# howardlau1999/pytorch-ddp-template

Hardware: NVIDIA H100
Metric: samples/sec (whole box, device-timed, max over ranks) for ResNet-50 DDP at 1/2/4/8 H100 (higher is better)
Workload: dtype bf16; 1 GPU; model=resnet50, global_batch=32, per_gpu_batch=32, image_size=224, parallelism=dp1, loss=mse(dense one-hot target), optimizer=sgd lr1e-3 + clip_grad_norm 1000 + linear warmup/decay, transport=single, cuda_graph=True

## Files before the change

### b200ddp/csrc/batchnorm.cu

```cuda
#include "ops.h"
#include "drv.h"
#include "tc_primitives.cuh"

#include <algorithm>
#include <cstdlib>
#include <map>
#include <mutex>
#include <utility>

namespace b200 {
namespace {

constexpr int kBnThreads = 256;
constexpr int kVec = 8;

template <typename T> __device__ __forceinline__ void bn_load8(const T* p, float* f);
template <> __device__ __forceinline__ void bn_load8<__nv_bfloat16>(const __nv_bfloat16* p, float* f) {
  unpack8(*reinterpret_cast<const Bf16x8*>(p), f);
}
template <> __device__ __forceinline__ void bn_load8<float>(const float* p, float* f) {
  const float4 a = reinterpret_cast<const float4*>(p)[0], b = reinterpret_cast<const float4*>(p)[1];
  f[0] = a.x; f[1] = a.y; f[2] = a.z; f[3] = a.w; f[4] = b.x; f[5] = b.y; f[6] = b.z; f[7] = b.w;
}
template <typename T> __device__ __forceinline__ void bn_store8(T* p, const float* f);
// ... 233 lines not shown
  bn_wait_producer();
  if (cv * kVec >= C) return;
  bn_apply_rows<T>(x, residual, y, mask, scale, shift, C, cv, r0, r1, tyi, ty, relu);
}

template <typename T>
__device__ __forceinline__ void bn_bwd_apply_rows(const T* __restrict__ dy, const T* __restrict__ x, const unsigned char* __restrict__ y,
                                                  T* __restrict__ dx, T* __restrict__ dres, const float* __restrict__ save_mean,
                                                  const float* __restrict__ save_rstd, const float* __restrict__ gamma,
                                                  const float* __restrict__ coef, int C, int cv, int r0, int r1, int tyi, int ty, int relu);
template <typename T>
__device__ __forceinline__ void bn_bwd_apply_rows_coef(const T* __restrict__ dy, const T* __restrict__ x, const unsigned char* __restrict__ y,
                                                       T* __restrict__ dx, T* __restrict__ dres, const float* __restrict__ save_mean,
                                                       const float* __restrict__ save_rstd, const float* __restrict__ gamma,
                                                       const float* c1p, const float* c2p, int C, int cv, int r0, int r1, int tyi, int ty, int relu);

template <typename T, bool FUSED, bool PDL = false>
__global__ void __launch_bounds__(kBnThreads, 2) bn_bwd_reduce_kernel(const T* __restrict__ dy, const T* __restrict__ x, const unsigned char* __restrict__ y,
                                                                     int R, int C, int cvb, int ty, int relu, const float* __restrict__ save_mean,
                                                                     const float* __restrict__ save_rstd, float* __restrict__ partial,
                                                                     unsigned int* __restrict__ counters, float* __restrict__ dgamma,
                                                                     float* __restrict__ dbeta, float* __restrict__ coef ,
                                                                     const float* __restrict__ gamma, T* __restrict__ dx, T* __restrict__ dres) {
  extern __shared__ float smem[];
  __shared__ bool is_last;
  unsigned int* gen = counters + gridDim.x;
  unsigned int gen0 = 0;
  if (FUSED && threadIdx.x == 0) gen0 = *reinterpret_cast<volatile unsigned int*>(&gen[blockIdx.x]);
  const int tx = threadIdx.x % cvb, tyi = threadIdx.x / cvb;
  const int cv = blockIdx.x * cvb + tx;
  const int S = gridDim.y;
  const int rows_per = (R + S - 1) / S;
  const int r0 = blockIdx.y * rows_per, r1 = min(R, r0 + rows_per);
  float acc[2][kVec];
#pragma unroll
  for (int i = 0; i < kVec; ++i) { acc[0][i] = 0.f; acc[1][i] = 0.f; }
  if (cv * kVec < C) {
    float mean[kVec], rstd[kVec];
    bn_load8<float>(save_mean + cv * kVec, mean);
    bn_load8<float>(save_rstd + cv * kVec, rstd);
    const size_t col = (size_t)cv * kVec;
    int r = r0 + tyi;
    for (; r + ty < r1; r += 2 * ty) {
      float g[2][kVec], xv[2][kVec];
      unsigned int mk[2] = {0xffu, 0xffu};
#pragma unroll
      for (int u = 0; u < 2; ++u) {
        const size_t off = (size_t)(r + u * ty) * C + col;
        bn_load8<T>(dy + off, g[u]);
        bn_load8<T>(x + off, xv[u]);
        if (relu) mk[u] = y[(size_t)(r + u * ty) * (C / kVec) + cv];
      }
#pragma unroll
      for (int u = 0; u < 2; ++u)
#pragma unroll
        for (int i = 0; i < kVec; ++i) {
          const float gm = ((mk[u] >> i) & 1u) ? g[u][i] : 0.f;
          acc[0][i] += gm;
          acc[1][i] = fmaf(gm, (xv[u][i] - mean[i]) * rstd[i], acc[1][i]);
        }
    }
    for (; r < r1; r += ty) {
      float g[kVec], xv[kVec];
      const size_t off = (size_t)r * C + col;
      bn_load8<T>(dy + off, g);
      bn_load8<T>(x + off, xv);
      const unsigned int mk = relu ? y[(size_t)r * (C / kVec) + cv] : 0xffu;
#pragma unroll
      for (int i = 0; i < kVec; ++i) {
        const float gm = ((mk >> i) & 1u) ? g[i] : 0.f;
        acc[0][i] += gm;
        acc[1][i] = fmaf(gm, (xv[i] - mean[i]) * rstd[i], acc[1][i]);
      }
    }
  }
  if constexpr (PDL) bn_launch_dependents();
  reduce_rows<2>(acc, smem, tx, tyi, cvb, ty);
  const int width = cvb * kVec;
  const int c0 = blockIdx.x * width;
  for (int c = threadIdx.x; c < width; c += blockDim.x) {
    if (c0 + c < C) {
      partial[(size_t)(0 * S + blockIdx.y) * C + c0 + c] = smem[c];
      partial[(size_t)(1 * S + blockIdx.y) * C + c0 + c] = smem[ty * width + c];
    }
  }
  __threadfence();
  __syncthreads();
  if (threadIdx.x == 0) {
    const unsigned int ticket = atomicAdd(&counters[blockIdx.x], 1u);
    is_last = (ticket == (unsigned int)S - 1);
  }
  __syncthreads();
  if (!FUSED && !is_last) return;
  if (is_last) {
    __threadfence();
    const float inv_r = 1.f / (float)R;
    const int lanes = max(1, (int)blockDim.x / width);
    {
      const int c = threadIdx.x % width, l = threadIdx.x / width;
      float ps = 0.f, pq = 0.f;
      if (l < lanes && c0 + c < C) {
  #pragma unroll 4
        for (int k = l; k < S; k += lanes) { ps += __ldcg(&partial[(size_t)(0 * S + k) * C + c0 + c]); pq += __ldcg(&partial[(size_t)(1 * S + k) * C + c0 + c]); }
      }
      __syncthreads();
      if (l < lanes) { smem[l * width + c] = ps; smem[(lanes + l) * width + c] = pq; }
      __syncthreads();
    }
    for (int c = threadIdx.x; c < width; c += blockDim.x) {
      const int ch = c0 + c;
      if (ch >= C) continue;
      float s = 0.f, q = 0.f;
      for (int l = 0; l < lanes; ++l) { s += smem[l * width + c]; q += smem[(lanes + l) * width + c]; }
      dbeta[ch] = s;
      dgamma[ch] = q;
      coef[ch] = s * inv_r;
      coef[C + ch] = q * inv_r;
    }

    __syncthreads();
    if (threadIdx.x == 0) {
      counters[blockIdx.x] = 0u;
      if (FUSED) { __threadfence(); bn_st_release(&gen[blockIdx.x], gen0 + 1u); }
    }
  }
  if (!FUSED) return;
  if (!is_last && threadIdx.x == 0) bn_wait_generation(&gen[blockIdx.x], gen0);
  __syncthreads();
  if (cv * kVec < C) bn_bwd_apply_rows<T>(dy, x, y, dx, dres, save_mean, save_rstd, gamma, coef, C, cv, r0, r1, tyi, ty, relu);
}

template <typename T>
__device__ __forceinline__ void bn_bwd_apply_rows_coef(const T* __restrict__ dy, const T* __restrict__ x, const unsigned char* __restrict__ y,
                                                       T* __restrict__ dx, T* __restrict__ dres, const float* __restrict__ save_mean,
                                                       const float* __restrict__ save_rstd, const float* __restrict__ gamma,
                                                       const float* c1p, const float* c2p, int C, int cv, int r0, int r1, int tyi, int ty, int relu) {
  float ka[kVec], kb[kVec], kc[kVec];
  {
    float mean[kVec], rstd[kVec], gam[kVec], c1[kVec], c2[kVec];
    bn_load8<float>(save_mean + cv * kVec, mean);
    bn_load8<float>(save_rstd + cv * kVec, rstd);
    bn_load8<float>(gamma + cv * kVec, gam);
    bn_load8<float>(c1p, c1);
    bn_load8<float>(c2p, c2);
#pragma unroll
    for (int i = 0; i < kVec; ++i) {
      ka[i] = gam[i] * rstd[i];
      kb[i] = -ka[i] * rstd[i] * c2[i];
      kc[i] = -ka[i] * (c1[i] - mean[i] * rstd[i] * c2[i]);
    }
  }
  const size_t col = (size_t)cv * kVec;
  int r = r0 + tyi;
  for (; r + ty < r1; r += 2 * ty) {
    float g[2][kVec], xv[2][kVec];
    unsigned int mk[2] = {0xffu, 0xffu};
#pragma unroll
    for (int u = 0; u < 2; ++u) {
      const size_t off = (size_t)(r + u * ty) * C + col;
      bn_load8<T>(dy + off, g[u]);
      bn_load8<T>(x + off, xv[u]);
      if (relu) mk[u] = y[(size_t)(r + u * ty) * (C / kVec) + cv];
    }
#pragma unroll
    for (int u = 0; u < 2; ++u) {
      const size_t off = (size_t)(r + u * ty) * C + col;
      float o[kVec];
#pragma unroll
      for (int i = 0; i < kVec; ++i) {
        if (!((mk[u] >> i) & 1u)) g[u][i] = 0.f;
        o[i] = fmaf(ka[i], g[u][i], fmaf(kb[i], xv[u][i], kc[i]));
      }
      if (dres != nullptr) bn_store8<T>(dres + off, g[u]);
      bn_store8<T>(dx + off, o);
    }
  }
  for (; r < r1; r += ty) {
    const size_t off = (size_t)r * C + col;
    float g[kVec], xv[kVec], o[kVec];
    bn_load8<T>(dy + off, g);
    bn_load8<T>(x + off, xv);
    const unsigned int mk = relu ? y[(size_t)r * (C / kVec) + cv] : 0xffu;
#pragma unroll
    for (int i = 0; i < kVec; ++i) {
      if (!((mk >> i) & 1u)) g[i] = 0.f;
      o[i] = fmaf(ka[i], g[i], fmaf(kb[i], xv[i], kc[i]));
    }
    if (dres != nullptr) bn_store8<T>(dres + off, g);
    bn_store8<T>(dx + off, o);
  }
}

template <typename T>
__device__ __forceinline__ void bn_bwd_apply_rows(const T* __restrict__ dy, const T* __restrict__ x, const unsigned char* __restrict__ y,
                                                  T* __restrict__ dx, T* __restrict__ dres, const float* __restrict__ save_mean,
                                                  const float* __restrict__ save_rstd, const float* __restrict__ gamma,
                                                  const float* __restrict__ coef, int C, int cv, int r0, int r1, int tyi, int ty, int relu) {
  bn_bwd_apply_rows_coef<T>(dy, x, y, dx, dres, save_mean, save_rstd, gamma, coef + cv * kVec, coef + C + cv * kVec, C, cv, r0, r1, tyi, ty, relu);
}

template <typename T>
__global__ void __launch_bounds__(kBnThreads) bn_bwd_apply_kernel(const T* __restrict__ dy, const T* __restrict__ x, const unsigned char* __restrict__ y,
                                                                 T* __restrict__ dx, T* __restrict__ dres, const float* __restrict__ save_mean,
                                                                 const float* __restrict__ save_rstd, const float* __restrict__ gamma,
                                                                 const float* __restrict__ coef, int R, int C, int cvb, int ty, int relu) {
  const int tx = threadIdx.x % cvb, tyi = threadIdx.x / cvb;
  const int cv = blockIdx.x * cvb + tx;
  if (cv * kVec >= C) return;
  const int S = gridDim.y;
  const int rows_per = (R + S - 1) / S;
  const int r0 = blockIdx.y * rows_per, r1 = min(R, r0 + rows_per);
  bn_bwd_apply_rows<T>(dy, x, y, dx, dres, save_mean, save_rstd, gamma, coef, C, cv, r0, r1, tyi, ty, relu);
}

template <typename T>
__global__ void __launch_bounds__(kBnThreads) bn_bwd_apply_pdl_kernel(const T* __restrict__ dy, const T* __restrict__ x, const unsigned char* __restrict__ y,
                                                                     T* __restrict__ dx, T* __restrict__ dres, const float* __restrict__ save_mean,
                                                                     const float* __restrict__ save_rstd, const float* __restrict__ gamma,
                                                                     const float* __restrict__ coef, int R, int C, int cvb, int ty, int relu) {
  const int tx = threadIdx.x % cvb, tyi = threadIdx.x / cvb;
  const int cv = blockIdx.x * cvb + tx;
  const int S = gridDim.y;
  const int rows_per = (R + S - 1) / S;
  const int r0 = blockIdx.y * rows_per, r1 = min(R, r0 + rows_per);
  bn_wait_producer();
  if (cv * kVec >= C) return;
  bn_bwd_apply_rows<T>(dy, x, y, dx, dres, save_mean, save_rstd, gamma, coef, C, cv, r0, r1, tyi, ty, relu);
}

int g_bn_pdl = -1;
bool bn_pdl_enabled() {
  if (g_bn_pdl < 0) { const char* e = getenv("B200DDP_PDL"); g_bn_pdl = (e && atoi(e) != 0) ? 1 : 0; }
  return g_bn_pdl > 0;
}

template <typename... KArgs, typename... Args>
void launch_dependent(void (*kernel)(KArgs...), dim3 grid, cudaStream_t s, Args... args) {
  cudaLaunchConfig_t cfg = {};
  cfg.gridDim = grid;
  cfg.blockDim = dim3(kBnThreads);
  cfg.dynamicSmemBytes = 0;
  cfg.stream = s;
  cudaLaunchAttribute attr[1];
  attr[0].id = cudaLaunchAttributeProgrammaticStreamSerialization;
  attr[0].val.programmaticStreamSerializationAllowed = 1;
  cfg.attrs = attr;
  cfg.numAttrs = 1;
  B200_CUDA_CHECK(cudaLaunchKernelEx(&cfg, kernel, static_cast<KArgs>(args)...));
}

Tile pick_tile(int R, int C) {
  Tile t;
  const int cv = C / kVec;
  t.cvb = cv < 8 ? cv : 8;
  while (kBnThreads % t.cvb != 0) --t.cvb;
  t.ty = kBnThreads / t.cvb;
  t.grid_x = (cv + t.cvb - 1) / t.cvb;
  int want = (4 * kNumSMs + t.grid_x - 1) / t.grid_x;
  int max_by_rows = R / (t.ty * 4);
  if (max_by_rows < 1) max_by_rows = 1;
  t.grid_y = want < max_by_rows ? want : max_by_rows;
  if (t.grid_y > 256) t.grid_y = 256;
  return t;
}

dim3 apply_grid(const Tile& t, int R) {
  int want = (8 * kNumSMs + t.grid_x - 1) / t.grid_x;
  int max_by_rows = R / (t.ty * 4);
  if (max_by_rows < 1) max_by_rows = 1;
  int gy = want < max_by_rows ? want : max_by_rows;
  return dim3(t.grid_x, gy);
}

bool fused_tile(int R, int C, Tile* t) {
  static int enabled = -1;
  if (enabled < 0) { const char* e = getenv("B200DDP_BN_FUSED"); enabled = (e && atoi(e) == 1) ? 1 : 0; }
  *t = pick_tile(R, C);
  if (!enabled || t->grid_x > 2 * kNumSMs) return false;
  int cap = (2 * kNumSMs) / t->grid_x;
  if (cap < 1) cap = 1;
  if (t->grid_y > cap) t->grid_y = cap;
  return true;
}

constexpr int kResThreads = 256;
constexpr int kResTile = 64;
constexpr int kResMaxBox = 256;
constexpr int kResMaxBoxes = 16;
constexpr int kResWarps = kResThreads / 32;
constexpr int kResMaxWaves = 2;
constexpr int kResFixedSmem = kResMaxBoxes * 8 + (kResWarps * 2 + 2 + 3) * kResTile * 4;

__device__ unsigned int g_bn_resident_error = 0;

struct ResGeom {
  int R, C;
  int T;
  int P;
  int box_rows;
  int nbox;
  int waves;
};

__device__ __forceinline__ void res_grid_sync(unsigned int* bar, unsigned int nblocks) {
  __syncthreads();
  if (threadIdx.x == 0) {
    unsigned int* gen = bar + 1;
    const unsigned int g0 = bn_ld_acquire(gen);
    __threadfence();
    if (atomicAdd(bar, 1u) == nblocks - 1) {
      atomicExch(bar, 0u);
      __threadfence();
      bn_st_release(gen, g0 + 1u);
    } else {
      unsigned long long t0;
      asm volatile("mov.u64 %0, %%globaltimer;" : "=l"(t0));
      while (bn_ld_acquire(gen) == g0) {
        unsigned long long t;
        asm volatile("mov.u64 %0, %%globaltimer;" : "=l"(t));
        if (t - t0 > 2000000000ull) { atomicExch(&g_bn_resident_error, 1u); break; }
      }
    }
    __threadfence();
  }
  __syncthreads();
}

__device__ __forceinline__ void res_write_partials(float (&acc)[2][kVec], float* red, float* __restrict__ partial, int P, int p, int C,
                                                   int c0) {
  const int lane = threadIdx.x & 31, warp = threadIdx.x >> 5, cv = threadIdx.x & 7;
#pragma unroll
  for (int a = 0; a < 2; ++a)
#pragma unroll
    for (int i = 0; i < kVec; ++i) {
      float v = acc[a][i];
      v += __shfl_xor_sync(0xffffffffu, v, 8);
      v += __shfl_xor_sync(0xffffffffu, v, 16);
      if (lane < 8) red[(warp * 2 + a) * kResTile + cv * kVec + i] = v;
    }
  __syncthreads();
  if (threadIdx.x < 2 * kResTile) {
    const int a = threadIdx.x / kResTile, c = threadIdx.x % kResTile;
    float s = 0.f;
    for (int w = 0; w < kResWarps; ++w) s += red[(w * 2 + a) * kResTile + c];
    if (c0 + c < C) partial[((size_t)a * P + p) * C + c0 + c] = s;
  }
}

__device__ __forceinline__ void res_reduce_partials(float* red, const float* __restrict__ partial, int P, int C, int c0) {
  const int q = threadIdx.x & 31, l = threadIdx.x >> 5;
  const int a = q >> 4, c4 = (q & 15) * 4;
  float4 s = make_float4(0.f, 0.f, 0.f, 0.f);
  if (c0 + c4 < C) {
    const float* base = partial + (size_t)a * P * C + c0 + c4;
#pragma unroll 4
    for (int k = l; k < P; k += kResWarps) {
      const float4 v = __ldcg(reinterpret_cast<const float4*>(base + (size_t)k * C));
      s.x += v.x; s.y += v.y; s.z += v.z; s.w += v.w;
    }
  }
  __syncthreads();
  *reinterpret_cast<float4*>(red + (l * 2 + a) * kResTile + c4) = s;
  __syncthreads();
  if (threadIdx.x < 2 * kResTile) {
    const int aa = threadIdx.x / kResTile, c = threadIdx.x % kResTile;
    float t = 0.f;
    for (int w = 0; w < kResWarps; ++w) t += red[(w * 2 + aa) * kResTile + c];
    red[kResWarps * 2 * kResTile + aa * kResTile + c] = t;
  }
  __syncthreads();
}

__device__ __forceinline__ void res_ld8(const unsigned char* s, float* f) { unpack8(*reinterpret_cast<const Bf16x8*>(s), f); }
__device__ __forceinline__ void res_st8(unsigned char* s, const float* f) { *reinterpret_cast<Bf16x8*>(s) = pack8(f); }

__global__ void __launch_bounds__(kResThreads, 2)
bn_resident_fwd_kernel(const __grid_constant__ CUtensorMap map_x, const __grid_constant__ CUtensorMap map_y,
                       const __grid_constant__ CUtensorMap map_res, const __nv_bfloat16* __restrict__ residual, unsigned char* __restrict__ mask, const float* __restrict__ gamma,
                       const float* __restrict__ beta, float* __restrict__ running_mean, float* __restrict__ running_var,
                       long long* __restrict__ num_batches, float* __restrict__ save_mean, float* __restrict__ save_rstd,
                       float* __restrict__ scale, float* __restrict__ shift, float* __restrict__ partial, unsigned int* __restrict__ bar,
                       float eps, float momentum, int relu, const ResGeom g) {
  extern __shared__ __align__(128) unsigned char res_smem[];
  const int slab_rows = g.nbox * g.box_rows;
  const uint32_t box_bytes = (uint32_t)g.box_rows * kResTile * 2;
  unsigned char* data = res_smem;
  uint64_t* mbar = reinterpret_cast<uint64_t*>(res_smem + (size_t)slab_rows * kResTile * 2);
  float* red = reinterpret_cast<float*>(mbar + kResMaxBoxes);
  float* coef = red + kResWarps * 2 * kResTile + 2 * kResTile;
  const int cv = threadIdx.x & 7, rl = threadIdx.x >> 3;
  const int ntiles = (g.C + kResTile - 1) / kResTile, cvs = g.C / kVec;
  const int slot = blockIdx.x / g.P, p = blockIdx.x % g.P;
  const int r0 = p * slab_rows;
  const int nlive = r0 >= g.R ? 0 : min(g.nbox, (g.R - r0 + g.box_rows - 1) / g.box_rows);
  if (threadIdx.x == 0) {
    for (int b = 0; b < g.nbox; ++b) tc::mbar_init(&mbar[b], 1);
    asm volatile("fence.mbarrier_init.release.cluster;" ::: "memory");
    tc::tma_prefetch_desc(&map_x);
    tc::tma_prefetch_desc(&map_y);
    if (blockIdx.x == 0 && num_batches != nullptr) *num_batches += 1;
  }
  __syncthreads();
  for (int w = 0; w < g.waves; ++w) {
    const int t = w * g.T + slot;
    const bool active = t < ntiles;
    const int c0 = t * kResTile;
    const int cvg = t * (kResTile / kVec) + cv;
    if (active && threadIdx.x == 0) {
      for (int b = 0; b < nlive; ++b) {
        tc::mbar_expect_tx(&mbar[b], box_bytes);
        tc::tma_load_2d(&map_x, &mbar[b], data + (size_t)b * box_bytes, c0, r0 + b * g.box_rows);
      }
    }
    float acc[2][kVec];
#pragma unroll
    for (int i = 0; i < kVec; ++i) { acc[0][i] = 0.f; acc[1][i] = 0.f; }
    if (active) {
      for (int b = 0; b < nlive; ++b) {
        tc::mbar_wait(&mbar[b], (uint32_t)(w & 1));
        const unsigned char* box = data + (size_t)b * box_bytes + cv * 16;
        for (int rr = rl; rr < g.box_rows; rr += 4 * 32) {
          float f[4][kVec];
#pragma unroll
          for (int u = 0; u < 4; ++u) {
            if (rr + u * 32 < g.box_rows) res_ld8(box + (size_t)(rr + u * 32) * (kResTile * 2), f[u]);
            else
#pragma unroll
              for (int i = 0; i < kVec; ++i) f[u][i] = 0.f;
          }
#pragma unroll
          for (int u = 0; u < 4; ++u)
#pragma unroll
            for (int i = 0; i < kVec; ++i) { acc[0][i] += f[u][i]; acc[1][i] = fmaf(f[u][i], f[u][i], acc[1][i]); }
        }
      }
      if (residual != nullptr && threadIdx.x == 0) {
        for (int b = 0; b < nlive; ++b)
          asm volatile("cp.async.bulk.prefetch.tensor.2d.L2.global [%0, {%1, %2}];"
                       ::"l"(reinterpret_cast<uint64_t>(&map_res)), "r"(c0), "r"(r0 + b * g.box_rows) : "memory");
      }
      res_write_partials(acc, red, partial, g.P, p, g.C, c0);
    }
    res_grid_sync(bar, gridDim.x);
    if (!active) continue;
    res_reduce_partials(red, partial, g.P, g.C, c0);
    if (threadIdx.x < kResTile) {
      const float* tot = red + kResWarps * 2 * kResTile;
      const int c = threadIdx.x, ch = c0 + c;
      if (ch < g.C) {
        const float inv_r = 1.f / (float)g.R;
        const float mean = tot[c] * inv_r;
        const float var = fmaxf(tot[kResTile + c] * inv_r - mean * mean, 0.f);
        const float rstd = rsqrtf(var + eps);
        const float sc = gamma[ch] * rstd;
        const float sh = beta[ch] - mean * sc;
        coef[c] = sc;
        coef[kResTile + c] = sh;
        if (p == 0) {
          save_mean[ch] = mean;
          save_rstd[ch] = rstd;
          scale[ch] = sc;
          shift[ch] = sh;
          if (running_mean != nullptr) {
            const float unbiased = g.R > 1 ? var * ((float)g.R / (float)(g.R - 1)) : var;
            running_mean[ch] = (1.f - momentum) * running_mean[ch] + momentum * mean;
            running_var[ch] = (1.f - momentum) * running_var[ch] + momentum * unbiased;
          }
        }
      } else {
        coef[c] = 0.f;
        coef[kResTile + c] = 0.f;
      }
    }
    __syncthreads();
    float sc[kVec], sh[kVec];
#pragma unroll
    for (int i = 0; i < kVec; ++i) { sc[i] = coef[cv * kVec + i]; sh[i] = coef[kResTile + cv * kVec + i]; }
    const bool live_cv = cvg < cvs;
    for (int b = 0; b < nlive; ++b) {
      unsigned char* box = data + (size_t)b * box_bytes + cv * 16;
      const int rb = r0 + b * g.box_rows;
      for (int rr = rl; rr < g.box_rows; rr += 8 * 32) {
        Bf16x8 rv[8];
#pragma unroll
        for (int u = 0; u < 8; ++u) {
          const int r = rb + rr + u * 32;
          if (residual != nullptr && rr + u * 32 < g.box_rows && r < g.R && live_cv)
            rv[u] = *reinterpret_cast<const Bf16x8*>(residual + (size_t)r * g.C + (size_t)cvg * kVec);
        }
#pragma unroll
        for (int u = 0; u < 8; ++u) {
          const int r = rb + rr + u * 32;
          if (!(rr + u * 32 < g.box_rows && r < g.R && live_cv)) continue;
          float f[kVec], rs[kVec];
          res_ld8(box + (size_t)(rr + u * 32) * (kResTile * 2), f);
          if (residual != nullptr) unpack8(rv[u], rs);
          unsigned int bits = 0;
#pragma unroll
          for (int i = 0; i < kVec; ++i) {
            float v = fmaf(f[i], sc[i], sh[i]);
            if (residual != nullptr) v += rs[i];
            bits |= (v > 0.f ? 1u : 0u) << i;
            f[i] = relu ? fmaxf(v, 0.f) : v;
          }
          res_st8(box + (size_t)(rr + u * 32) * (kResTile * 2), f);
          if (mask != nullptr) mask[(size_t)r * cvs + cvg] = (unsigned char)bits;
        }
      }
      tc::fence_async_smem();
      __syncthreads();
      if (threadIdx.x == 0) { tc::tma_store_2d(&map_y, data + (size_t)b * box_bytes, c0, rb); tc::bulk_commit(); }
    }
    if (threadIdx.x == 0) asm volatile("cp.async.bulk.wait_group.read 0;" ::: "memory");
    __syncthreads();
  }
  if (threadIdx.x == 0) tc::bulk_wait_all();
}

__global__ void __launch_bounds__(kResThreads, 2)
bn_resident_bwd_kernel(const __grid_constant__ CUtensorMap map_dy, const __grid_constant__ CUtensorMap map_x,
                       const __grid_constant__ CUtensorMap map_dx, const __grid_constant__ CUtensorMap map_dres,
                       const unsigned char* __restrict__ mask, const float* __restrict__ save_mean, const float* __restrict__ save_rstd,
                       const float* __restrict__ gamma, float* __restrict__ dgamma, float* __restrict__ dbeta, float* __restrict__ coef_out,
                       float* __restrict__ partial, unsigned int* __restrict__ bar, int relu, int want_dres, const ResGeom g) {
  extern __shared__ __align__(128) unsigned char res_smem[];
  const int slab_rows = g.nbox * g.box_rows;
  const uint32_t box_bytes = (uint32_t)g.box_rows * kResTile * 2;
  unsigned char* dyd = res_smem;
  unsigned char* xd = res_smem + (size_t)slab_rows * kResTile * 2;
  uint64_t* mbar = reinterpret_cast<uint64_t*>(res_smem + (size_t)2 * slab_rows * kResTile * 2);
  float* red = reinterpret_cast<float*>(mbar + kResMaxBoxes);
  float* coef = red + kResWarps * 2 * kResTile + 2 * kResTile;
  unsigned char* smask = reinterpret_cast<unsigned char*>(coef + 3 * kResTile);
  const int cv = threadIdx.x & 7, rl = threadIdx.x >> 3;
  const int ntiles = (g.C + kResTile - 1) / kResTile, cvs = g.C / kVec;
  const int slot = blockIdx.x / g.P, p = blockIdx.x % g.P;
  const int r0 = p * slab_rows;
  const int nlive = r0 >= g.R ? 0 : min(g.nbox, (g.R - r0 + g.box_rows - 1) / g.box_rows);
  if (threadIdx.x == 0) {
    for (int b = 0; b < g.nbox; ++b) tc::mbar_init(&mbar[b], 1);
    asm volatile("fence.mbarrier_init.release.cluster;" ::: "memory");
    tc::tma_prefetch_desc(&map_dy);
    tc::tma_prefetch_desc(&map_x);
  }
  __syncthreads();
  for (int w = 0; w < g.waves; ++w) {
    const int t = w * g.T + slot;
    const bool active = t < ntiles;
    const int c0 = t * kResTile;
    const int cvg = t * (kResTile / kVec) + cv;
    const bool live_cv = cvg < cvs;
    if (active && threadIdx.x == 0) {
      for (int b = 0; b < nlive; ++b) {
        tc::mbar_expect_tx(&mbar[b], 2 * box_bytes);
        tc::tma_load_2d(&map_dy, &mbar[b], dyd + (size_t)b * box_bytes, c0, r0 + b * g.box_rows);
        tc::tma_load_2d(&map_x, &mbar[b], xd + (size_t)b * box_bytes, c0, r0 + b * g.box_rows);
      }
    }
    if (active && relu) {
      const int n = min(slab_rows, g.R - r0) * 8;
#pragma unroll 8
      for (int i = threadIdx.x; i < n; i += kResThreads) {
        const int cg = t * (kResTile / kVec) + (i & 7);
        smask[i] = cg < cvs ? mask[(size_t)(r0 + (i >> 3)) * cvs + cg] : 0u;
      }
      __syncthreads();
    }
    float acc[2][kVec];
#pragma unroll
    for (int i = 0; i < kVec; ++i) { acc[0][i] = 0.f; acc[1][i] = 0.f; }
    if (active) {
      float mean[kVec], rstd[kVec];
#pragma unroll
      for (int i = 0; i < kVec; ++i) { mean[i] = 0.f; rstd[i] = 0.f; }
      if (live_cv) { bn_load8<float>(save_mean + cvg * kVec, mean); bn_load8<float>(save_rstd + cvg * kVec, rstd); }
      for (int b = 0; b < nlive; ++b) {
        tc::mbar_wait(&mbar[b], (uint32_t)(w & 1));
        for (int rr = rl; rr < g.box_rows; rr += 2 * 32) {
          float gv[2][kVec], xv[2][kVec];
          unsigned int mk[2];
#pragma unroll
          for (int u = 0; u < 2; ++u) {
            const int q = min(rr + u * 32, g.box_rows - 1);
            res_ld8(dyd + (size_t)b * box_bytes + (size_t)q * (kResTile * 2) + cv * 16, gv[u]);
            res_ld8(xd + (size_t)b * box_bytes + (size_t)q * (kResTile * 2) + cv * 16, xv[u]);
            mk[u] = rr + u * 32 < g.box_rows ? (relu ? smask[(b * g.box_rows + q) * 8 + cv] : 0xffu) : 0u;
          }
#pragma unroll
          for (int u = 0; u < 2; ++u)
#pragma unroll
            for (int i = 0; i < kVec; ++i) {
              const float gm = ((mk[u] >> i) & 1u) ? gv[u][i] : 0.f;
              acc[0][i] += gm;
              acc[1][i] = fmaf(gm, (xv[u][i] - mean[i]) * rstd[i], acc[1][i]);
            }
        }
      }
      res_write_partials(acc, red, partial, g.P, p, g.C, c0);
    }
    res_grid_sync(bar, gridDim.x);
    if (!active) continue;
    res_reduce_partials(red, partial, g.P, g.C, c0);
    if (threadIdx.x < kResTile) {
      const float* tot = red + kResWarps * 2 * kResTile;
      const int c = threadIdx.x, ch = c0 + c;
      float ka = 0.f, kb = 0.f, kc = 0.f;
      if (ch < g.C) {
        const float inv_r = 1.f / (float)g.R;
        const float s1 = tot[c], s2 = tot[kResTile + c];
        const float c1 = s1 * inv_r, c2 = s2 * inv_r;
        const float mean = save_mean[ch], rstd = save_rstd[ch];
        ka = gamma[ch] * rstd;
        kb = -ka * rstd * c2;
        kc = -ka * (c1 - mean * rstd * c2);
        if (p == 0) {
          dbeta[ch] = s1;
          dgamma[ch] = s2;
          coef_out[ch] = c1;
          coef_out[g.C + ch] = c2;
        }
      }
      coef[c] = ka;
      coef[kResTile + c] = kb;
      coef[2 * kResTile + c] = kc;
    }
    __syncthreads();
    float ka[kVec], kb[kVec], kc[kVec];
#pragma unroll
    for (int i = 0; i < kVec; ++i) {
      ka[i] = coef[cv * kVec + i];
      kb[i] = coef[kResTile + cv * kVec + i];
      kc[i] = coef[2 * kResTile + cv * kVec + i];
    }
    for (int b = 0; b < nlive; ++b) {
      const int rb = r0 + b * g.box_rows;
      unsigned char* gbox = dyd + (size_t)b * box_bytes + cv * 16;
      unsigned char* xbox = xd + (size_t)b * box_bytes + cv * 16;
      for (int rr = rl; rr < g.box_rows; rr += 2 * 32) {
        float gv[2][kVec], xv[2][kVec];
        unsigned int mk[2];
#pragma unroll
        for (int u = 0; u < 2; ++u) {
          const int q = min(rr + u * 32, g.box_rows - 1);
          res_ld8(gbox + (size_t)q * (kResTile * 2), gv[u]);
          res_ld8(xbox + (size_t)q * (kResTile * 2), xv[u]);
          mk[u] = relu ? smask[(b * g.box_rows + q) * 8 + cv] : 0xffu;
        }
#pragma unroll
        for (int u = 0; u < 2; ++u) {
          if (rr + u * 32 >= g.box_rows) continue;
          const size_t off = (size_t)(rr + u * 32) * (kResTile * 2);
          float o[kVec];
#pragma unroll
          for (int i = 0; i < kVec; ++i) {
            if (!((mk[u] >> i) & 1u)) gv[u][i] = 0.f;
            o[i] = fmaf(ka[i], gv[u][i], fmaf(kb[i], xv[u][i], kc[i]));
          }
          if (want_dres) res_st8(gbox + off, gv[u]);
          res_st8(xbox + off, o);
        }
      }
      tc::fence_async_smem();
      __syncthreads();
      if (threadIdx.x == 0) {
        tc::tma_store_2d(&map_dx, xd + (size_t)b * box_bytes, c0, rb);
        if (want_dres) tc::tma_store_2d(&map_dres, dyd + (size_t)b * box_bytes, c0, rb);
        tc::bulk_commit();
      }
    }
    if (threadIdx.x == 0) asm volatile("cp.async.bulk.wait_group.read 0;" ::: "memory");
    __syncthreads();
  }
  if (threadIdx.x == 0) tc::bulk_wait_all();
}

int g_bn_two_pass = 0;

bool resident_allowed() {
  static int fused_env = -1;
  if (fused_env < 0) { const char* e = getenv("B200DDP_BN_FUSED"); fused_env = (e && atoi(e) == 1) ? 1 : 0; }
  return !g_bn_two_pass && !fused_env && !bn_pdl_enabled();
}

struct ResPlan {
  bool ok = false;
  ResGeom g{};
  int grid = 0;
  int smem = 0;
};

ResPlan resident_plan(int R, int C, int streams) {
  static std::mutex mu;
  static std::map<std::pair<int, std::pair<long long, int>>, ResPlan> cache;
  int dev = 0;
  B200_CUDA_CHECK(cudaGetDevice(&dev));
  const auto key = std::make_pair(dev, std::make_pair(((long long)R << 20) | (long long)C, streams));
  std::lock_guard<std::mutex> lock(mu);
  auto it = cache.find(key);
  if (it != cache.end()) return it->second;
  ResPlan plan;
  int sms = 0, optin = 0;
  B200_CUDA_CHECK(cudaDeviceGetAttribute(&sms, cudaDevAttrMultiProcessorCount, dev));
  B200_CUDA_CHECK(cudaDeviceGetAttribute(&optin, cudaDevAttrMaxSharedMemoryPerBlockOptin, dev));
  const long long budget = (long long)optin - kResFixedSmem - 1024;
  const int ntiles = (C + kResTile - 1) / kResTile;
  const long long row_bytes = (long long)kResTile * 2 * streams + (streams == 2 ? 8 : 0);
  for (int T = ntiles; T >= 1 && R > 0; --T) {
    int P = sms / T;
    if (P < 1) continue;
    P = std::min(P, std::max(1, (R + 31) / 32));
    const int need = (R + P - 1) / P;
    const int nbox = (need + kResMaxBox - 1) / kResMaxBox;
    if (nbox > kResMaxBoxes) continue;
    const int box_rows = (need + nbox - 1) / nbox;
    const long long slab = (long long)nbox * box_rows * row_bytes;
    if (slab > budget) continue;
    if ((ntiles + T - 1) / T > kResMaxWaves) break;
    plan.g = ResGeom{R, C, T, (R + nbox * box_rows - 1) / (nbox * box_rows), box_rows, nbox, (ntiles + T - 1) / T};
    plan.grid = plan.g.T * plan.g.P;
    plan.smem = (int)slab + kResFixedSmem;
    plan.ok = true;
    break;
  }
  cache.emplace(key, plan);
  return plan;
}

CUtensorMap res_map(const void* ptr, int R, int C, int box_rows) {
  auto& drv = Driver::get();
  if (!drv.TensorMapEncodeTiled) throw std::runtime_error("batch norm: cuTensorMapEncodeTiled unavailable");
  CUtensorMap map;
  cuuint64_t dims[2] = {(cuuint64_t)C, (cuuint64_t)R};
  cuuint64_t strides[1] = {(cuuint64_t)C * 2};
  cuuint32_t box[2] = {(cuuint32_t)kResTile, (cuuint32_t)box_rows};
  cuuint32_t es[2] = {1, 1};
  B200_DRV_CHECK(drv.TensorMapEncodeTiled(&map, CU_TENSOR_MAP_DATA_TYPE_BFLOAT16, 2, const_cast<void*>(ptr), dims, strides, box, es,
                                          CU_TENSOR_MAP_INTERLEAVE_NONE, CU_TENSOR_MAP_SWIZZLE_NONE, CU_TENSOR_MAP_L2_PROMOTION_L2_256B,
                                          CU_TENSOR_MAP_FLOAT_OOB_FILL_NONE));
  return map;
}

int res_smem_limit() {
  int dev = 0, optin = 0;
  B200_CUDA_CHECK(cudaGetDevice(&dev));
  B200_CUDA_CHECK(cudaDeviceGetAttribute(&optin, cudaDevAttrMaxSharedMemoryPerBlockOptin, dev));
  return optin;
}

bool res_aligned(const void* p) { return p == nullptr || (reinterpret_cast<uintptr_t>(p) & 15u) == 0; }

template <typename... KArgs, typename... Args>
void launch_cooperative(void (*kernel)(KArgs...), const ResPlan& plan, cudaStream_t s, Args... args) {
  cudaLaunchConfig_t cfg = {};
  cfg.gridDim = dim3(plan.grid);
  cfg.blockDim = dim3(kResThreads);
  cfg.dynamicSmemBytes = plan.smem;
  cfg.stream = s;
  cudaLaunchAttribute attr[1];
  attr[0].id = cudaLaunchAttributeCooperative;
  attr[0].val.cooperative = 1;
  cfg.attrs = attr;
  cfg.numAttrs = 1;
  B200_CUDA_CHECK(cudaLaunchKernelEx(&cfg, kernel, static_cast<KArgs>(args)...));
}

}

template <typename T>
__global__ void __launch_bounds__(kBnThreads) bn_apply_partials_kernel(const T* __restrict__ x, const T* __restrict__ residual, T* __restrict__ y,
                                                                      unsigned char* __restrict__ mask, const float* __restrict__ partial, int G,
                                                                      const float* __restrict__ gamma, const float* __restrict__ beta,
                                                                      float* __restrict__ running_mean, float* __restrict__ running_var,
                                                                      long long* __restrict__ num_batches, float* __restrict__ save_mean,
                                                                      float* __restrict__ save_rstd, float eps, float momentum, int R, int C,
                                                                      int cvb, int ty, int relu) {
  extern __shared__ float bn_smem[];
  const int tx = threadIdx.x % cvb, tyi = threadIdx.x / cvb;
  const int cv = blockIdx.x * cvb + tx;
  const bool live = cv * kVec < C;
  float acc[2][kVec];
#pragma unroll
  for (int i = 0; i < kVec; ++i) { acc[0][i] = 0.f; acc[1][i] = 0.f; }
  if (live) {
    for (int g = tyi; g < G; g += ty) {
      float a[kVec], b[kVec];
      bn_load8<float>(partial + (size_t)g * C + cv * kVec, a);
      bn_load8<float>(partial + ((size_t)G + g) * C + cv * kVec, b);
#pragma unroll
      for (int i = 0; i < kVec; ++i) { acc[0][i] += a[i]; acc[1][i] += b[i]; }
    }
  }
  reduce_rows<2>(acc, bn_smem, tx, tyi, cvb, ty);
  const int width = cvb * kVec;
  float* sc_s = bn_smem + 2 * ty * width;
  float* sh_s = sc_s + width;
  if (tyi == 0 && live) {
    const float inv_r = 1.f / (float)R;
#pragma unroll
    for (int i = 0; i < kVec; ++i) {
      const int ch = cv * kVec + i;
      const float sum = bn_smem[tx * kVec + i], sq = bn_smem[ty * width + tx * kVec + i];
      const float mean = sum * inv_r;
      const float var = fmaxf(sq * inv_r - mean * mean, 0.f);
      const float rstd = rsqrtf(var + eps);
      const float sc = gamma[ch] * rstd;
      sc_s[tx * kVec + i] = sc;
      sh_s[tx * kVec + i] = beta[ch] - mean * sc;
      if (blockIdx.y == 0) {
        save_mean[ch] = mean;
        save_rstd[ch] = rstd;
        if (running_mean != nullptr) {
          const float unbiased = R > 1 ? var * ((float)R / (float)(R - 1)) : var;
          running_mean[ch] = (1.f - momentum) * running_mean[ch] + momentum * mean;
          running_var[ch] = (1.f - momentum) * running_var[ch] + momentum * unbiased;
        }
      }
    }
  }
  if (blockIdx.x == 0 && blockIdx.y == 0 && threadIdx.x == 0 && num_batches != nullptr) *num_batches += 1;
  __syncthreads();
  if (!live) return;
  const int S = gridDim.y;
  const int rows_per = (R + S - 1) / S;
  const int r0 = blockIdx.y * rows_per, r1 = min(R, r0 + rows_per);
  bn_apply_rows<T>(x, residual, y, mask, sc_s - (size_t)blockIdx.x * width, sh_s - (size_t)blockIdx.x * width, C, cv, r0, r1, tyi, ty, relu);
}

template <typename T>
__global__ void __launch_bounds__(kBnThreads) bn_bwd_apply_partials_kernel(const T* __restrict__ dy, const T* __restrict__ x, const unsigned char* __restrict__ y,
                                                                          T* __restrict__ dx, T* __restrict__ dres, const float* __restrict__ partial, int G,
                                                                          const float* __restrict__ save_mean, const float* __restrict__ save_rstd,
                                                                          const float* __restrict__ gamma, float* __restrict__ dgamma,
                                                                          float* __restrict__ dbeta, int R, int C, int cvb, int ty, int relu) {
  extern __shared__ float bn_smem[];
  const int tx = threadIdx.x % cvb, tyi = threadIdx.x / cvb;
  const int cv = blockIdx.x * cvb + tx;
  const bool live = cv * kVec < C;
  float acc[2][kVec];
#pragma unroll
  for (int i = 0; i < kVec; ++i) { acc[0][i] = 0.f; acc[1][i] = 0.f; }
  if (live) {
    for (int g = tyi; g < G; g += ty) {
      float a[kVec], b[kVec];
      bn_load8<float>(partial + (size_t)g * C + cv * kVec, a);
      bn_load8<float>(partial + ((size_t)G + g) * C + cv * kVec, b);
#pragma unroll
      for (int i = 0; i < kVec; ++i) { acc[0][i] += a[i]; acc[1][i] += b[i]; }
    }
  }
  reduce_rows<2>(acc, bn_smem, tx, tyi, cvb, ty);
  const int width = cvb * kVec;
  float* c1_s = bn_smem + 2 * ty * width;
  float* c2_s = c1_s + width;
  if (tyi == 0 && live) {
    const float inv_r = 1.f / (float)R;
#pragma unroll
    for (int i = 0; i < kVec; ++i) {
      const int ch = cv * kVec + i;
      const float s1 = bn_smem[tx * kVec + i], s2 = bn_smem[ty * width + tx * kVec + i];
      c1_s[tx * kVec + i] = s1 * inv_r;
      c2_s[tx * kVec + i] = s2 * inv_r;
      if (blockIdx.y == 0) { dgamma[ch] = s2; dbeta[ch] = s1; }
    }
  }
  __syncthreads();
  if (!live) return;
  const int S = gridDim.y;
  const int rows_per = (R + S - 1) / S;
  const int r0 = blockIdx.y * rows_per, r1 = min(R, r0 + rows_per);
  bn_bwd_apply_rows_coef<T>(dy, x, y, dx, dres, save_mean, save_rstd, gamma, c1_s + tx * kVec, c2_s + tx * kVec, C, cv, r0, r1, tyi, ty, relu);
}

void set_bn_pdl(int on) { g_bn_pdl = on; }

void set_bn_two_pass(int on) { g_bn_two_pass = on ? 1 : 0; }

unsigned int bn_resident_error() {
  unsigned int v = 0;
  B200_CUDA_CHECK(cudaMemcpyFromSymbol(&v, g_bn_resident_error, sizeof(v)));
  return v;
}

void bn_workspace_sizes(int R, int C, size_t* partial_floats, size_t* counters) {
  const Tile t = pick_tile(R, C);
  const ResPlan fwd = resident_plan(R, C, 1), bwd = resident_plan(R, C, 2);
  const int p = std::max(fwd.ok ? fwd.g.P : 0, bwd.ok ? bwd.g.P : 0);
  *partial_floats = (size_t)2 * std::max(t.grid_y, p) * C;
  *counters = (size_t)2 * t.grid_x + 2;
}

void launch_bn_forward(const void* x, const void* residual, void* y, unsigned char* mask, DType dt, int R, int C, const float* gamma, const float* beta,
                       float* running_mean, float* running_var, long long* num_batches, float* save_mean, float* save_rstd,
                       float* scale, float* shift, float* partial, unsigned int* counters, float eps, float momentum, bool relu,
                       cudaStream_t s) {
  if (C % kVec != 0) throw std::runtime_error("fused batch norm: channel count must be a multiple of 8");
  const int r = relu ? 1 : 0;
  if (dt == DType::BF16 && resident_allowed() && res_aligned(x) && res_aligned(residual) && res_aligned(y)) {
    const ResPlan plan = resident_plan(R, C, 1);
    if (plan.ok) {
      static std::atomic<unsigned long long> smem_done{0};
      ensure_max_dynamic_smem(bn_resident_fwd_kernel, res_smem_limit(), smem_done);
      const CUtensorMap mx = res_map(x, R, C, plan.g.box_rows), my = res_map(y, R, C, plan.g.box_rows);
      const CUtensorMap mres = residual != nullptr ? res_map(residual, R, C, plan.g.box_rows) : mx;
      launch_cooperative(bn_resident_fwd_kernel, plan, s, mx, my, mres, (const __nv_bfloat16*)residual, mask, gamma, beta, running_mean, running_var,
                         num_batches, save_mean, save_rstd, scale, shift, partial, counters + 2 * pick_tile(R, C).grid_x, eps, momentum, r,
                         plan.g);
      B200_COUNT_LAUNCH(1);
      return;
    }
  }
  Tile t;
  const bool fused = fused_tile(R, C, &t);
  const size_t smem = (size_t)2 * t.ty * t.cvb * kVec * sizeof(float);
  const dim3 grid(t.grid_x, t.grid_y);
  if (!fused && bn_pdl_enabled()) {
#define B200_BN_FWD_PDL(T)                                                                                                                  \
    bn_stats_kernel<T, false, true><<<grid, kBnThreads, smem, s>>>((const T*)x, R, C, t.cvb, t.ty, partial, counters, gamma, beta, running_mean, \
                                                                   running_var, num_batches, save_mean, save_rstd, scale, shift, eps, momentum,  \
                                                                   (const T*)residual, (T*)y, mask, r);                                          \
    B200_CUDA_CHECK(cudaGetLastError()); B200_COUNT_LAUNCH(1);                                                                                   \
    launch_dependent(bn_apply_pdl_kernel<T>, apply_grid(t, R), s, (const T*)x, (const T*)residual, (T*)y, mask, (const float*)scale,              \
                     (const float*)shift, R, C, t.cvb, t.ty, r);                                                                                  \
    B200_COUNT_LAUNCH(1)
    if (dt == DType::BF16) { B200_BN_FWD_PDL(__nv_bfloat16); } else { B200_BN_FWD_PDL(float); }
#undef B200_BN_FWD_PDL
    return;
  }
#define B200_BN_FWD(T, F)                                                                                                            \
  bn_stats_kernel<T, F><<<grid, kBnThreads, smem, s>>>((const T*)x, R, C, t.cvb, t.ty, partial, counters, gamma, beta, running_mean, \
                                                       running_var, num_batches, save_mean, save_rstd, scale, shift, eps, momentum, \
                                                       (const T*)residual, (T*)y, mask, r)
  if (dt == DType::BF16) { if (fused) B200_BN_FWD(__nv_bfloat16, true); else B200_BN_FWD(__nv_bfloat16, false); }
  else { if (fused) B200_BN_FWD(float, true); else B200_BN_FWD(float, false); }
#undef B200_BN_FWD
  B200_CUDA_CHECK(cudaGetLastError()); B200_COUNT_LAUNCH(1);
  if (fused) return;
  if (dt == DType::BF16)
    bn_apply_kernel<__nv_bfloat16><<<apply_grid(t, R), kBnThreads, 0, s>>>((const __nv_bfloat16*)x, (const __nv_bfloat16*)residual,
                                                                           (__nv_bfloat16*)y, mask, scale, shift, R, C, t.cvb, t.ty, r);
  else
    bn_apply_kernel<float><<<apply_grid(t, R), kBnThreads, 0, s>>>((const float*)x, (const float*)residual, (float*)y, mask, scale, shift, R, C,
                                                                   t.cvb, t.ty, r);
  B200_CUDA_CHECK(cudaGetLastError()); B200_COUNT_LAUNCH(1);
}

void launch_bn_forward_from_partials(const void* x, const void* residual, void* y, unsigned char* mask, DType dt, int R, int C,
                                     const float* gamma, const float* beta, float* running_mean, float* running_var,
                                     long long* num_batches, float* save_mean, float* save_rstd, float* scale, float* shift,
                                     const float* partial, int groups, float eps, float momentum, bool relu, cudaStream_t s) {
  (void)scale; (void)shift;
  if (C % kVec != 0) throw std::runtime_error("fused batch norm: channel count must be a multiple of 8");
  if (groups < 1) throw std::runtime_error("fused batch norm: empty partial statistics");
  const Tile t = pick_tile(R, C);
  const int r = relu ? 1 : 0;
  const size_t smem = (size_t)(2 * t.ty + 2) * t.cvb * kVec * sizeof(float);
  if (dt == DType::BF16)
    bn_apply_partials_kernel<__nv_bfloat16><<<apply_grid(t, R), kBnThreads, smem, s>>>(
        (const __nv_bfloat16*)x, (const __nv_bfloat16*)residual, (__nv_bfloat16*)y, mask, partial, groups, gamma, beta, running_mean, running_var,
        num_batches, save_mean, save_rstd, eps, momentum, R, C, t.cvb, t.ty, r);
  else
    bn_apply_partials_kernel<float><<<apply_grid(t, R), kBnThreads, smem, s>>>(
        (const float*)x, (const float*)residual, (float*)y, mask, partial, groups, gamma, beta, running_mean, running_var, num_batches, save_mean,
        save_rstd, eps, momentum, R, C, t.cvb, t.ty, r);
  B200_CUDA_CHECK(cudaGetLastError()); B200_COUNT_LAUNCH(1);
}

void launch_bn_backward_from_partials(const void* dy, const void* x, const void* y, void* dx, void* dres, DType dt, int R, int C, const float* gamma,
                                      const float* save_mean, const float* save_rstd, float* dgamma, float* dbeta, const float* partial, int groups,
                                      bool relu, cudaStream_t s) {
  if (C % kVec != 0) throw std::runtime_error("fused batch norm: channel count must be a multiple of 8");
  if (groups < 1) throw std::runtime_error("fused batch norm: empty partial sums");
  const Tile t = pick_tile(R, C);
  const int r = relu ? 1 : 0;
  const size_t smem = (size_t)(2 * t.ty + 2) * t.cvb * kVec * sizeof(float);
  if (dt == DType::BF16)
    bn_bwd_apply_partials_kernel<__nv_bfloat16><<<apply_grid(t, R), kBnThreads, smem, s>>>(
        (const __nv_bfloat16*)dy, (const __nv_bfloat16*)x, (const unsigned char*)y, (__nv_bfloat16*)dx, (__nv_bfloat16*)dres, partial, groups, save_mean,
        save_rstd, gamma, dgamma, dbeta, R, C, t.cvb, t.ty, r);
  else
    bn_bwd_apply_partials_kernel<float><<<apply_grid(t, R), kBnThreads, smem, s>>>(
        (const float*)dy, (const float*)x, (const unsigned char*)y, (float*)dx, (float*)dres, partial, groups, save_mean, save_rstd, gamma, dgamma, dbeta,
        R, C, t.cvb, t.ty, r);
  B200_CUDA_CHECK(cudaGetLastError()); B200_COUNT_LAUNCH(1);
}

void launch_bn_backward(const void* dy, const void* x, const void* y, void* dx, void* dres, DType dt, int R, int C, const float* gamma,
                        const float* save_mean, const float* save_rstd, float* dgamma, float* dbeta, float* coef, float* partial,
                        unsigned int* counters, bool relu, cudaStream_t s) {
  if (C % kVec != 0) throw std::runtime_error("fused batch norm: channel count must be a multiple of 8");
  const int r = relu ? 1 : 0;
  if (dt == DType::BF16 && resident_allowed() && res_aligned(dy) && res_aligned(x) && res_aligned(dx) && res_aligned(dres)) {
    const ResPlan plan = resident_plan(R, C, 2);
    if (plan.ok) {
      static std::atomic<unsigned long long> smem_done{0};
      ensure_max_dynamic_smem(bn_resident_bwd_kernel, res_smem_limit(), smem_done);
      const int br = plan.g.box_rows;
      const CUtensorMap mdy = res_map(dy, R, C, br), mx = res_map(x, R, C, br), mdx = res_map(dx, R, C, br);
      const CUtensorMap mdres = dres != nullptr ? res_map(dres, R, C, br) : mdx;
      launch_cooperative(bn_resident_bwd_kernel, plan, s, mdy, mx, mdx, mdres, (const unsigned char*)y, save_mean, save_rstd, gamma, dgamma,
                         dbeta, coef, partial, counters + 2 * pick_tile(R, C).grid_x, r, dres != nullptr ? 1 : 0, plan.g);
      B200_COUNT_LAUNCH(1);
      return;
    }
  }
  Tile t;
  const bool fused = fused_tile(R, C, &t);
  const size_t smem = (size_t)2 * t.ty * t.cvb * kVec * sizeof(float);
  const dim3 grid(t.grid_x, t.grid_y);
  if (!fused && bn_pdl_enabled()) {
#define B200_BN_BWD_PDL(T)                                                                                                                   \
    bn_bwd_reduce_kernel<T, false, true><<<grid, kBnThreads, smem, s>>>((const T*)dy, (const T*)x, (const unsigned char*)y, R, C, t.cvb, t.ty, r,  \
                                                                        save_mean, save_rstd, partial, counters, dgamma, dbeta, coef, gamma,      \
                                                                        (T*)dx, (T*)dres);                                                        \
    B200_CUDA_CHECK(cudaGetLastError()); B200_COUNT_LAUNCH(1);                                                                                     \
    launch_dependent(bn_bwd_apply_pdl_kernel<T>, apply_grid(t, R), s, (const T*)dy, (const T*)x, (const unsigned char*)y, (T*)dx, (T*)dres,         \
                     save_mean, save_rstd, gamma, (const float*)coef, R, C, t.cvb, t.ty, r);                                                        \
    B200_COUNT_LAUNCH(1)
    if (dt == DType::BF16) { B200_BN_BWD_PDL(__nv_bfloat16); } else { B200_BN_BWD_PDL(float); }
#undef B200_BN_BWD_PDL
    return;
  }
#define B200_BN_BWD(T, F)                                                                                                              \
  bn_bwd_reduce_kernel<T, F><<<grid, kBnThreads, smem, s>>>((const T*)dy, (const T*)x, (const unsigned char*)y, R, C, t.cvb, t.ty, r,  \
                                                            save_mean, save_rstd, partial, counters, dgamma, dbeta, coef, gamma,      \
                                                            (T*)dx, (T*)dres)
  if (dt == DType::BF16) { if (fused) B200_BN_BWD(__nv_bfloat16, true); else B200_BN_BWD(__nv_bfloat16, false); }
  else { if (fused) B200_BN_BWD(float, true); else B200_BN_BWD(float, false); }
#undef B200_BN_BWD
  B200_CUDA_CHECK(cudaGetLastError()); B200_COUNT_LAUNCH(1);
  if (fused) return;
  if (dt == DType::BF16)
    bn_bwd_apply_kernel<__nv_bfloat16><<<apply_grid(t, R), kBnThreads, 0, s>>>((const __nv_bfloat16*)dy, (const __nv_bfloat16*)x, (const unsigned char*)y,
                                                                               (__nv_bfloat16*)dx, (__nv_bfloat16*)dres, save_mean, save_rstd, gamma, coef,
                                                                               R, C, t.cvb, t.ty, r);
  else
    bn_bwd_apply_kernel<float><<<apply_grid(t, R), kBnThreads, 0, s>>>((const float*)dy, (const float*)x, (const unsigned char*)y, (float*)dx,
                                                                       (float*)dres, save_mean, save_rstd, gamma, coef, R, C, t.cvb, t.ty, r);
  B200_CUDA_CHECK(cudaGetLastError()); B200_COUNT_LAUNCH(1);
}

}
```

Measured before the change: 4959 samples/s.

## Pipeline next-tile TMA loads and use per-tile barriers in resident batchnorm

Resident batchnorm kernels now prefetch the next channel tile's boxes via TMA as soon as each box's store has drained, instead of loading at the start of each wave. The grid-wide barrier is replaced with a per-channel-tile barrier over only the P blocks sharing a tile, so tiles no longer wait on each other. The counter workspace grows to hold two words per tile. The risks are extra barrier-slot bookkeeping and ordering hazards between the async store reads and the reloads into the same shared-memory boxes.

Measured after the change: 5024 samples/s (median of 6 runs). +1.3%, better.

```diff
diff --git a/b200ddp/csrc/batchnorm.cu b/b200ddp/csrc/batchnorm.cu
--- a/b200ddp/csrc/batchnorm.cu
+++ b/b200ddp/csrc/batchnorm.cu
@@ -559,7 +559,7 @@
   int waves;
 };
 
-__device__ __forceinline__ void res_grid_sync(unsigned int* bar, unsigned int nblocks) {
+__device__ __forceinline__ void res_tile_sync(unsigned int* bar, unsigned int nblocks) {
   __syncthreads();
   if (threadIdx.x == 0) {
     unsigned int* gen = bar + 1;
@@ -650,56 +650,54 @@
   const int slot = blockIdx.x / g.P, p = blockIdx.x % g.P;
   const int r0 = p * slab_rows;
   const int nlive = r0 >= g.R ? 0 : min(g.nbox, (g.R - r0 + g.box_rows - 1) / g.box_rows);
+  auto load_box = [&](int tile, int b) {
+    tc::mbar_expect_tx(&mbar[b], box_bytes);
+    tc::tma_load_2d(&map_x, &mbar[b], data + (size_t)b * box_bytes, tile * kResTile, r0 + b * g.box_rows);
+  };
   if (threadIdx.x == 0) {
     for (int b = 0; b < g.nbox; ++b) tc::mbar_init(&mbar[b], 1);
     asm volatile("fence.mbarrier_init.release.cluster;" ::: "memory");
     tc::tma_prefetch_desc(&map_x);
     tc::tma_prefetch_desc(&map_y);
     if (blockIdx.x == 0 && num_batches != nullptr) *num_batches += 1;
+    if (slot < ntiles)
+      for (int b = 0; b < nlive; ++b) load_box(slot, b);
   }
   __syncthreads();
   for (int w = 0; w < g.waves; ++w) {
     const int t = w * g.T + slot;
-    const bool active = t < ntiles;
+    if (t >= ntiles) break;
+    const bool more = t + g.T < ntiles;
     const int c0 = t * kResTile;
     const int cvg = t * (kResTile / kVec) + cv;
-    if (active && threadIdx.x == 0) {
-      for (int b = 0; b < nlive; ++b) {
-        tc::mbar_expect_tx(&mbar[b], box_bytes);
-        tc::tma_load_2d(&map_x, &mbar[b], data + (size_t)b * box_bytes, c0, r0 + b * g.box_rows);
-      }
-    }
     float acc[2][kVec];
 #pragma unroll
     for (int i = 0; i < kVec; ++i) { acc[0][i] = 0.f; acc[1][i] = 0.f; }
-    if (active) {
-      for (int b = 0; b < nlive; ++b) {
-        tc::mbar_wait(&mbar[b], (uint32_t)(w & 1));
-        const unsigned char* box = data + (size_t)b * box_bytes + cv * 16;
-        for (int rr = rl; rr < g.box_rows; rr += 4 * 32) {
-          float f[4][kVec];
-#pragma unroll
-          for (int u = 0; u < 4; ++u) {
-            if (rr + u * 32 < g.box_rows) res_ld8(box + (size_t)(rr + u * 32) * (kResTile * 2), f[u]);
-            else
-#pragma unroll
-              for (int i = 0; i < kVec; ++i) f[u][i] = 0.f;
-          }
-#pragma unroll
-          for (int u = 0; u < 4; ++u)
-#pragma unroll
-            for (int i = 0; i < kVec; ++i) { acc[0][i] += f[u][i]; acc[1][i] = fmaf(f[u][i], f[u][i], acc[1][i]); }
+    for (int b = 0; b < nlive; ++b) {
+      tc::mbar_wait(&mbar[b], (uint32_t)(w & 1));
+      const unsigned char* box = data + (size_t)b * box_bytes + cv * 16;
+      for (int rr = rl; rr < g.box_rows; rr += 4 * 32) {
+        float f[4][kVec];
+#pragma unroll
+        for (int u = 0; u < 4; ++u) {
+          if (rr + u * 32 < g.box_rows) res_ld8(box + (size_t)(rr + u * 32) * (kResTile * 2), f[u]);
+          else
+#pragma unroll
+            for (int i = 0; i < kVec; ++i) f[u][i] = 0.f;
         }
-      }
-      if (residual != nullptr && threadIdx.x == 0) {
-        for (int b = 0; b < nlive; ++b)
-          asm volatile("cp.async.bulk.prefetch.tensor.2d.L2.global [%0, {%1, %2}];"
-                       ::"l"(reinterpret_cast<uint64_t>(&map_res)), "r"(c0), "r"(r0 + b * g.box_rows) : "memory");
-      }
-      res_write_partials(acc, red, partial, g.P, p, g.C, c0);
-    }
-    res_grid_sync(bar, gridDim.x);
-    if (!active) continue;
+#pragma unroll
+        for (int u = 0; u < 4; ++u)
+#pragma unroll
+          for (int i = 0; i < kVec; ++i) { acc[0][i] += f[u][i]; acc[1][i] = fmaf(f[u][i], f[u][i], acc[1][i]); }
+      }
+    }
+    if (residual != nullptr && threadIdx.x == 0) {
+      for (int b = 0; b < nlive; ++b)
+        asm volatile("cp.async.bulk.prefetch.tensor.2d.L2.global [%0, {%1, %2}];"
+                     ::"l"(reinterpret_cast<uint64_t>(&map_res)), "r"(c0), "r"(r0 + b * g.box_rows) : "memory");
+    }
+    res_write_partials(acc, red, partial, g.P, p, g.C, c0);
+    res_tile_sync(bar + 2 * slot, g.P);
     res_reduce_partials(red, partial, g.P, g.C, c0);
     if (threadIdx.x < kResTile) {
       const float* tot = red + kResWarps * 2 * kResTile;
@@ -766,9 +764,16 @@
       }
       tc::fence_async_smem();
       __syncthreads();
-      if (threadIdx.x == 0) { tc::tma_store_2d(&map_y, data + (size_t)b * box_bytes, c0, rb); tc::bulk_commit(); }
-    }
-    if (threadIdx.x == 0) asm volatile("cp.async.bulk.wait_group.read 0;" ::: "memory");
+      if (threadIdx.x == 0) {
+        tc::tma_store_2d(&map_y, data + (size_t)b * box_bytes, c0, rb);
+        tc::bulk_commit();
+        if (more && b > 0) { tc::bulk_wait_read_le1(); load_box(t + g.T, b - 1); }
+      }
+    }
+    if (threadIdx.x == 0 && more && nlive > 0) {
+      asm volatile("cp.async.bulk.wait_group.read 0;" ::: "memory");
+      load_box(t + g.T, nlive - 1);
+    }
     __syncthreads();
   }
   if (threadIdx.x == 0) tc::bulk_wait_all();
@@ -794,27 +799,29 @@
   const int slot = blockIdx.x / g.P, p = blockIdx.x % g.P;
   const int r0 = p * slab_rows;
   const int nlive = r0 >= g.R ? 0 : min(g.nbox, (g.R - r0 + g.box_rows - 1) / g.box_rows);
+  auto load_box = [&](int tile, int b) {
+    const int c0 = tile * kResTile, rb = r0 + b * g.box_rows;
+    tc::mbar_expect_tx(&mbar[b], 2 * box_bytes);
+    tc::tma_load_2d(&map_dy, &mbar[b], dyd + (size_t)b * box_bytes, c0, rb);
+    tc::tma_load_2d(&map_x, &mbar[b], xd + (size_t)b * box_bytes, c0, rb);
+  };
   if (threadIdx.x == 0) {
     for (int b = 0; b < g.nbox; ++b) tc::mbar_init(&mbar[b], 1);
     asm volatile("fence.mbarrier_init.release.cluster;" ::: "memory");
     tc::tma_prefetch_desc(&map_dy);
     tc::tma_prefetch_desc(&map_x);
+    if (slot < ntiles)
+      for (int b = 0; b < nlive; ++b) load_box(slot, b);
   }
   __syncthreads();
   for (int w = 0; w < g.waves; ++w) {
     const int t = w * g.T + slot;
-    const bool active = t < ntiles;
+    if (t >= ntiles) break;
+    const bool more = t + g.T < ntiles;
     const int c0 = t * kResTile;
     const int cvg = t * (kResTile / kVec) + cv;
     const bool live_cv = cvg < cvs;
-    if (active && threadIdx.x == 0) {
-      for (int b = 0; b < nlive; ++b) {
-        tc::mbar_expect_tx(&mbar[b], 2 * box_bytes);
-        tc::tma_load_2d(&map_dy, &mbar[b], dyd + (size_t)b * box_bytes, c0, r0 + b * g.box_rows);
-        tc::tma_load_2d(&map_x, &mbar[b], xd + (size_t)b * box_bytes, c0, r0 + b * g.box_rows);
-      }
-    }
-    if (active && relu) {
+    if (relu) {
       const int n = min(slab_rows, g.R - r0) * 8;
 #pragma unroll 8
       for (int i = threadIdx.x; i < n; i += kResThreads) {
@@ -826,12 +833,13 @@
     float acc[2][kVec];
 #pragma unroll
     for (int i = 0; i < kVec; ++i) { acc[0][i] = 0.f; acc[1][i] = 0.f; }
-    if (active) {
+    {
       float mean[kVec], rstd[kVec];
 #pragma unroll
       for (int i = 0; i < kVec; ++i) { mean[i] = 0.f; rstd[i] = 0.f; }
       if (live_cv) { bn_load8<float>(save_mean + cvg * kVec, mean); bn_load8<float>(save_rstd + cvg * kVec, rstd); }
       for (int b = 0; b < nlive; ++b) {
+        const unsigned char* gbox = dyd + (size_t)b * box_bytes + cv * 16;
         tc::mbar_wait(&mbar[b], (uint32_t)(w & 1));
         for (int rr = rl; rr < g.box_rows; rr += 2 * 32) {
           float gv[2][kVec], xv[2][kVec];
@@ -839,7 +847,7 @@
 #pragma unroll
           for (int u = 0; u < 2; ++u) {
             const int q = min(rr + u * 32, g.box_rows - 1);
-            res_ld8(dyd + (size_t)b * box_bytes + (size_t)q * (kResTile * 2) + cv * 16, gv[u]);
+            res_ld8(gbox + (size_t)q * (kResTile * 2), gv[u]);
             res_ld8(xd + (size_t)b * box_bytes + (size_t)q * (kResTile * 2) + cv * 16, xv[u]);
             mk[u] = rr + u * 32 < g.box_rows ? (relu ? smask[(b * g.box_rows + q) * 8 + cv] : 0xffu) : 0u;
           }
@@ -853,10 +861,9 @@
             }
         }
       }
-      res_write_partials(acc, red, partial, g.P, p, g.C, c0);
-    }
-    res_grid_sync(bar, gridDim.x);
-    if (!active) continue;
+    }
+    res_write_partials(acc, red, partial, g.P, p, g.C, c0);
+    res_tile_sync(bar + 2 * slot, g.P);
     res_reduce_partials(red, partial, g.P, g.C, c0);
     if (threadIdx.x < kResTile) {
       const float* tot = red + kResWarps * 2 * kResTile;
@@ -923,9 +930,13 @@
         tc::tma_store_2d(&map_dx, xd + (size_t)b * box_bytes, c0, rb);
         if (want_dres) tc::tma_store_2d(&map_dres, dyd + (size_t)b * box_bytes, c0, rb);
         tc::bulk_commit();
-      }
-    }
-    if (threadIdx.x == 0) asm volatile("cp.async.bulk.wait_group.read 0;" ::: "memory");
+        if (more && b > 0) { tc::bulk_wait_read_le1(); load_box(t + g.T, b - 1); }
+      }
+    }
+    if (threadIdx.x == 0 && more && nlive > 0) {
+      asm volatile("cp.async.bulk.wait_group.read 0;" ::: "memory");
+      load_box(t + g.T, nlive - 1);
+    }
     __syncthreads();
   }
   if (threadIdx.x == 0) tc::bulk_wait_all();
@@ -1143,7 +1154,8 @@
   const ResPlan fwd = resident_plan(R, C, 1), bwd = resident_plan(R, C, 2);
   const int p = std::max(fwd.ok ? fwd.g.P : 0, bwd.ok ? bwd.g.P : 0);
   *partial_floats = (size_t)2 * std::max(t.grid_y, p) * C;
-  *counters = (size_t)2 * t.grid_x + 2;
+  const int ntiles = (C + kResTile - 1) / kResTile;
+  *counters = (size_t)2 * t.grid_x + 2 * ntiles;
 }
 
 void launch_bn_forward(const void* x, const void* residual, void* y, unsigned char* mask, DType dt, int R, int C, const float* gamma, const float* beta,
```
